# yijingru/KG_Instance_Segmentation

Hardware: AMD Instinct MI355X
Metric: imgs/s (train fwd+bwd) at 512x512 (higher is better)
Workload: dtype forward: f32-tolerance, hi + lo f16 planes (22 significant bits), 3 MFMA products / backward: f16 single planes, 1 MFMA product; f16 MFMA, fp32 accumulate; 1 GPU; KGnet train step fwd(dec+seg)+4xDetectionLossAll+SEG_loss+bwd+Adam, batch 8/GPU 3x512x512, 300 boxes/img, full HIP path; precision_policy=fp32, global_batch=8, parallelism=dp1, loss_readback=every step (train.py:156), grad_overflow=False

## Files before the change

include/kgnet_hip.h:

```cpp
#ifndef KGNET_HIP_H
#define KGNET_HIP_H
#ifdef __cplusplus
extern "C" {
#endif

typedef struct kg_planes {
    int a_planes, a_pstride;
    int b_planes, b_pstride;
    int c_planes, c_pstride;
    int y_planes, y_pstride;
    int w_planes;
    int reserved_;
    const float* scale;
    const float* oscale;
} kg_planes_t;

int kg_rows_format(void);

const char* kg_last_error(void);
const char* kg_last_kernel(void);
int kg_version(void);
int kg_device_arch(char* out, int cap);
int kg_tr_probe(void* out_u16x256, void* stream);
int kg_f64_probe(const double* a, const double* b, double* out5n, int n, void* stream);

int kg_conv2d_igemm(const void* x, const void* w, const float* bias, void* y, float* y_f32, const void* res,
                    const void* mask, const int* rowdesc, int M, int H, int W, int OH, int OW, int cin_pad, int ldx,
                    int Cout, int ldy, int ldres, int ldmask, int K, int KH, int KW, int stride, int pad, int dil,
                    int mode, int relu, int f32_C, int tile, const kg_planes_t* planes, void* stream);
int kg_conv2d_halo(const void* x, const void* w, const float* bias, void* y, float* y_f32, const void* res,
                   const void* mask, int N, int H, int W, int cin_pad, int ldx, int Cout, int ldy, int ldres, int ldmask,
                   int K, int KS, int flip, int relu, int f32_C, int wc, const int* tiletab, int ntiles, int total_rows,
                   const kg_planes_t* planes, void* stream);
int kg_conv2d_halo_heads2(const void* x, const void* w, const float* bias64, const int* vmap, float* kp, float* sh, float* md,
                          int N, int H, int W, int C, int ldx, int K, int kp_sigmoid, const kg_planes_t* planes, void* stream);
int kg_conv3x3_c64(const void* x, const void* w, const float* bias, void* y, const void* res, const void* mask, int N, int H, int W,
                   int ldx, int Cout, int ldy, int ldres, int ldmask, int K, int flip, int relu, const int* tiletab16, int ntiles,
                   void* stream);
int kg_conv7_narrow(const void* x, const void* w, void* y, const void* mask, int N, int H, int W, int ldx, int chan_lo, int chan_slot, int Cout, int ldy,
                    int ldmask, int K, int flip, void* stream);
int kg_conv3x3_ws(const void* x, const void* w, const float* bias, void* y, int N, int H, int W, int ldx, int ldy, int K, int relu,
                  const int* tiletab8, int ntiles, const kg_planes_t* planes, void* stream);
int kg_conv1x1(const void* x, const void* w, const float* bias, void* y, const void* res, const void* mask, long M, int K,
               int wK, int ldx, int Cout, int ldy, int ldres, int ldmask, int relu, void* stream);
int kg_pack_weight(const float* w, void* dst, int Cout, int Cin, int KH, int KW, int K, int cin_pad, int row0, int c0,
                   int transposed, int x_planes, int w_planes, void* stream);
int kg_pack_weight_rows(const float* w, void* dst, int Cout, int Cin, int KH, int KW, int K, int cin_pad, const int* rowmap,
                        int c0, int x_planes, int w_planes, int tap_stride, void* stream);
int kg_pack_weight_narrow(const float* w, void* dst, int Cout, int Cin, int KH, int KW, int K, int row0, int c0, int tap_stride, int tap_pitch,
                          void* stream);
int kg_pack_weight_batch(const void* jobs, int njobs, int total_blocks, void* stream);
int kg_im2col_small(const void* x, void* out, int N, int H, int W, int OH, int OW, int KH, int KW, int stride, int pad, int cin,
                    int ldx, int Kpad, void* stream);
int kg_conv2d_wgrad(const void* x, const void* dy, float* dwp, const int* rowdesc, int M, int H, int W, int OH, int OW,
                    int ldx, int lddy, int Cin, int Cout, int cin_lim, int cout_lim, int KH, int KW, int stride, int pad,
                    int dil, int mode, int nsplit, long split_stride, const kg_planes_t* planes, void* stream);
int kg_conv2d_wgrad_halo(const void* x, const void* dy, float* dwp, int N, int H, int W, int ldx, int lddy, int Cin, int Cout,
                         int cin_lim, int cout_lim, int KS, int nsplit, long split_stride, const int* tiletab16, int ntiles,
                         float* dbp, const kg_planes_t* planes, void* stream);
int kg_bias_grad_final(const float* part, float* db, int nsplit, int C, int accumulate, void* stream);
int kg_wgrad_reduce(const float* part, float* grad_oihw, int Cout, int Cin, int KH, int KW, int nsplit, long split_stride,
                    int accumulate, void* stream);
int kg_wgrad_reduce_multi(const float* part, float* const* grads_oihw, const int* counts, int ngrads, int Cin, int KH, int KW,
                          int nsplit, long split_stride, int accumulate, void* stream);
int kg_wgrad_reduce_bias(const float* part, float* const* grads_oihw, const int* counts, int ngrads, int Cin, int KH, int KW,
                         int nsplit, long split_stride, int accumulate, const float* bias_part, float* db, int bias_C, void* stream);
int kg_wgrad_reduce_defer(int on);
int kg_wgrad_reduce_pending(void);
int kg_wgrad_reduce_flush(void* stream);
int kg_bias_grad(const void* dy, float* db, float* scratch, int scratch_floats, int M, int C, int ld, int accumulate,
                 void* stream);
int kg_set_wgrad_tr(int use_transpose_read);

int kg_img_pack(const float* img_nchw, void* out_rows8, int ldout, int N, int C, int H, int W, const kg_planes_t* planes, void* stream);
int kg_bn_stats_train(const void* x, int ldx, int M, int C, const float* gamma, const float* beta, float* running_mean,
                      float* running_var, float momentum, float eps, float* mean_out, float* invstd_out, float* scale,
                      float* shift, float* scratch, int scratch_floats, const kg_planes_t* planes, void* stream);
int kg_conv_stats_begin(float* part, long cap_floats);
int kg_conv_stats_end(int* nb);
int kg_bn_finalize_train(const float* part, int nb, int M, int C, const float* gamma, const float* beta, float* running_mean,
                         float* running_var, float momentum, float eps, float* mean_out, float* invstd_out, float* scale,
                         float* shift, void* stream);
int kg_bn_scale_shift_eval(int C, const float* gamma, const float* beta, const float* running_mean,
                           const float* running_var, float eps, float* scale, float* shift, void* stream);
int kg_bn_apply(const void* x, int ldx, const float* scale, const float* shift, const void* res, int ldres, void* y,
                int ldy, int M, int C, int relu, const kg_planes_t* planes, void* stream);
int kg_bn_bwd(const void* x, int ldx, const void* dy, int lddy, const float* gamma, const float* mean,
              const float* invstd, float* dgamma, float* dbeta, int accumulate, void* dx, int lddx, int M, int C,
              float* scratch, int scratch_floats, const float* parts, int nb_parts, const float* parts_scale,
              const kg_planes_t* planes, void* stream);
int kg_bn_bwd_frozen(const void* x, int ldx, const void* dy, int lddy, const float* scale, const float* running_mean,
                     const float* running_var, float eps, float* dgamma, float* dbeta, int accumulate, void* dx, int lddx,
                     int M, int C, float* scratch, int scratch_floats, const kg_planes_t* planes, void* stream);
int kg_conv_bstats_begin(float* part, long cap_floats, const void* x, int ldx, int x_planes, int x_pstride, const float* mean,
                         const float* invstd);
int kg_maxpool3s2_fwd(const void* x, int ldx, void* y, int ldy, void* argmax_u8, int N, int H, int W, int C, const kg_planes_t* planes, void* stream);
int kg_maxpool3s2_bwd(const void* x, int ldx, const void* dy, int lddy, void* dx, int lddx, const void* argmax_u8, int N, int H, int W, int C,
                      const kg_planes_t* planes, void* stream);
int kg_bilinear_fwd(const void* x, int ldx, void* y, int ldy, int N, int IH, int IW, int OH, int OW, int C,
                    const int* boxdesc, const int* row2box, long total_out_rows, const kg_planes_t* planes, void* stream);
int kg_bilinear_bwd(const void* dy, int lddy, void* dx, int lddx, int N, int IH, int IW, int OH, int OW, int C,
                    const int* boxdesc, const int* row2box, long total_in_rows, const void* mask, int ldmask,
                    const kg_planes_t* planes, void* stream);
int kg_add_rows(const void* a, int lda, const void* b, int ldb, const void* mask, int ldm, void* y, int ldy, long M,
                int C, const float* scale, const float* scale2, const kg_planes_t* planes, void* stream);
int kg_sigmoid_inplace(float* x, long n, void* stream);
int kg_grad_pack(const float* g_nchw, const float* prob, void* out_rows, int N, int C, int H, int W, int ld, int cpad,
                 const kg_planes_t* planes, void* stream);
int kg_grad_pack3(const float* g0_nchw, const float* g1_nchw, const float* g2_nchw, const float* prob0, void* out_rows, int N, int C0, int C1, int C2,
                  int H, int W, int ld, int pad0, int pad1, int pad2, const kg_planes_t* planes, void* stream);

int kg_detection_loss_fwd(const float* kp, const float* sh, const float* md, const float* gt, int N, int H, int W,
                          float kp_radius, const float* den_override, float* scratch, int scratch_floats, float* out8,
                          void* stream);
int kg_detection_loss_bwd(const float* kp, const float* sh, const float* md, const float* gt, int N, int H, int W,
                          float kp_radius, const float* fin8, const float* grad_out, float* g_kp, float* g_sh,
                          float* g_md, void* stream);
int kg_seg_loss(const float* prob, const void* tgt_u8, const int* patches, const void* pairs, int npatches, float* part,
                float* out1, const float* grad_out, float* gprob, void* stream);

int kg_postproc_timing_begin(void);
int kg_postproc_timing_end(float* ms4);
long kg_postproc_workspace_bytes(int H, int W, int peak_cap, int skel_cap);
int kg_postproc_scale(const float* kp, const float* soff, const float* mid, int H, int W, double thresh, void* ws,
                      long ws_bytes, int peak_cap, int skel_cap, double* skel, int* nskel, double* heat_out,
                      double* blur_out, int* peaks_out, double* peak_conf_out, int* npeaks_out, void* stream);
int kg_skeleton_boxes(const double* skel, const int* nskel, int skel_cap, double scale, int do_refine, double* boxes,
                      int* nbox, int box_cap, void* stream);
int kg_nms(const double* boxes, const int* nbox, int box_cap, double thresh, void* ws, long ws_bytes, double* out,
           int* nkeep, void* stream);

long kg_postproc_batch_workspace_bytes(int N, int H, int W, int peak_cap, int skel_cap);
int kg_postproc_batch(const float* kp, const float* soff, const float* mid, int N, int H, int W, double thresh, void* ws,
                      long ws_bytes, int peak_cap, int skel_cap, double* skel, int* nskel, void* stream);
int kg_skeleton_boxes_batch(int N, int nscales, const double* const* skel, const int* const* nskel, const int* skel_cap,
                            const double* scale, int do_refine, double* boxes, int* nbox, int box_cap, void* stream);
long kg_nms_batch_workspace_bytes(int N, int box_cap);
int kg_nms_batch(int N, const double* boxes, const int* nbox, int box_cap, double thresh, void* ws, long ws_bytes, double* out,
                 int* nkeep, void* stream);

int kg_gt_maps(const float* kps, int n, int H, int W, float* out, void* stream);

int kg_sp_image(const void* imgs, int N, int H, int W, float* out, void* stream);
int kg_sp_warp_masks(const void* imgs, const int* inst_img, int ntot, int H, int W, void* out, int* box, void* stream);
int kg_sp_boxes(const void* imgs, int N, const int* box, int ntot, int kp_radius, int* counts, float* gtb, float* kp, int* keep,
                void* stream);

int kg_adam_step(const void* jobs, int njobs, int total_blocks, float beta1, float beta2, float eps, float step_size, float bc2_sqrt,
                 float weight_decay, void* stream);

int kg_host_crop_masks(const float* const* masks, const int* work, int nwork, int H, int W, unsigned char* out);
int kg_crop_masks(const void* masks, const int* work, int nwork, int H, int W, void* out, void* stream);
int kg_host_tile_table(const int* h, const int* w, const long* row0, int nb, int th, int tw, int* out, int cap);
int kg_host_bin_csr(const int* tab, int nb, int BS, int BY, int BX, int nbins, int* bin_start, int* bin_boxes, int cap);
int kg_host_match_boxes(const float* pb, int P, const float* gb, int G, int gstride, float thresh, int* pairs, int cap, int* count);

int kg_mask_areas(const void* masks, int n, long ld, int* area, void* stream);
int kg_mask_inter_pairs(const void* a, const void* b, const int* pairs, int npairs, long ld, int* inter, void* stream);

long kg_mask_bits_ld(int H, int W);
int kg_mask_pack_bits(const void* masks, int src_is_f32, int n, int H, int W, void* words, long ld_words, void* stream);
int kg_mask_unpack_bits(const void* words, long ld_words, int n, int H, int W, void* out, int out_is_u8, void* stream);
int kg_bitmask_areas(const void* words, int n, long ld_words, int* area, void* stream);
int kg_bitmask_inter_pairs(const void* a, int na, const void* b, int nb, const int* pairs, int npairs, long ld_words, int* inter,
                           void* stream);
int kg_instance_labels(const void* words, long ld_words, int n, const int* row_start, int nimg, int H, int W, const int* ids, int* labels,
                       long long* table, void* stream);
int kg_instance_overlay(const void* image, const void* words, long ld_words, int n, const int* row_start, int nimg, int H, int W,
                        const double* colors, double alpha, void* out, void* stream);

int kg_seg_build_rows(const int* boxtab8, int nb, int* rowdesc, int* row2box, int* srcrow, void* stream);
int kg_seg_build_rows_levels(int nlev, const int* const* boxtab8, const int* nb, int* const* rowdesc, int* const* row2box, int* const* srcrow,
                             void* stream);
int kg_rows_gather(const void* src, int ldsrc, const int* srcrow, void* dst, int lddst, long nrows, int C, void* stream);
int kg_rows_gather_planes(const void* src, int ldsrc, int src_pstride, const int* srcrow, void* dst, int lddst, int dst_pstride, long nrows, int C,
                          int P, void* stream);
int kg_seg_conv3_c1(const void* x, int ldx, int C, const float* w, const float* bias, const int* rowdesc, long M, float* y,
                    const kg_planes_t* planes, void* stream);
int kg_f32_to_bf16_rows(const float* acc, void* out, int C, long rows, int ldout, const void* addto, int ldadd,
                        void* stream);
int kg_rows_gather_f32(const float* src, int ldsrc, const int* srcrow, void* dst, int lddst, long nrows, int C,
                       const kg_planes_t* planes, void* stream);
int kg_planes_to_f32(const void* x, int ldx, float* out, int ldout, long rows, int C, const kg_planes_t* planes, void* stream);
int kg_f32_to_planes(const float* acc, int ldacc, void* out, int ldout, const void* addto, int ldadd, long rows, int C,
                     const kg_planes_t* planes, void* stream);
int kg_crop_grad_reduce(const void* ga, int lda, const void* gb, int ldb, long rows_a, const int* boxtab, const int* bin_start,
                        const int* bin_boxes, int bin_size, int N, int H, int W, int C, float* out, void* out_rows, int ldout,
                        const kg_planes_t* planes, void* stream);


int kg_mask_paste(const float* flat, const int* dets, int nd, int input_h, int input_w, int image_h, int image_w,
                  float seg_thresh, void* out, int out_is_u8, void* stream);
int kg_mask_paste_bits(const float* flat, const int* dets, int nd, int input_h, int input_w, int image_h, int image_w,
                       float seg_thresh, void* words, long ld_words, void* stream);

int kg_grad_scale(const void* const* ptrs, const void* const* probs, const long* counts, int n, int target_log2, void* scratch, float* out, void* stream);
int kg_scale_tensors(const void* jobs, int njobs, int total_blocks, int* nonfinite, void* stream);
int kg_rows_rescale(void* g, int ld, long M, int C, int target_log2, const float* cum_in, float* cum_out, float* r_out, void* scratch,
                    const kg_planes_t* planes, void* stream);
int kg_rows_scale(void* g, int ld, long M, int C, const float* r, const float* r2, const kg_planes_t* planes, void* stream);
int kg_rows_scale_multi(const long* desc, int n, const float* r, const float* r2, void* stream);

#ifdef __cplusplus
}
#endif
#endif
```

kg_instance_segmentation_amd/_lib.py:

```python
import ctypes
import os

_HERE = os.path.dirname(os.path.abspath(__file__))
LIB_PATH = os.environ.get("KG_LIB_PATH") or os.path.join(_HERE, "libkgnet_hip.so")
LIB_F16_PATH = os.environ.get("KG_LIB_F16_PATH") or os.path.join(os.path.dirname(LIB_PATH), "libkgnet_hip_f16.so")

c_int, c_long, c_float, c_double, c_void_p = ctypes.c_int, ctypes.c_long, ctypes.c_float, ctypes.c_double, ctypes.c_void_p
P = c_void_p

_SIGS = {
    "kg_version": [],
    "kg_rows_format": [],
    "kg_grad_scale": [P, P, P, c_int, c_int, P, P, P],
    "kg_scale_tensors": [P, c_int, c_int, P, P],
    "kg_rows_rescale": [P, c_int, c_long, c_int, c_int, P, P, P, P, P, P],
    "kg_rows_scale": [P, c_int, c_long, c_int, P, P, P, P],
    "kg_rows_scale_multi": [P, c_int, P, P, P],
    "kg_device_arch": [ctypes.c_char_p, c_int],
    "kg_tr_probe": [P, P],
    "kg_conv2d_igemm": [P, P, P, P, P, P, P, P] + [c_int] * 21 + [P, P],
    "kg_conv2d_halo": [P, P, P, P, P, P, P] + [c_int] * 15 + [P, c_int, c_int, P, P],
    "kg_conv1x1": [P, P, P, P, P, P, c_long] + [c_int] * 8 + [P],
    "kg_conv3x3_c64": [P, P, P, P, P, P] + [c_int] * 11 + [P, c_int, P],
    "kg_conv3x3_ws": [P, P, P, P] + [c_int] * 7 + [P, c_int, P, P],
    "kg_pack_weight": [P, P] + [c_int] * 11 + [P],
    "kg_pack_weight_rows": [P, P] + [c_int] * 6 + [P, c_int, c_int, c_int, c_int, P],
    "kg_pack_weight_batch": [P, c_int, c_int, P],
    "kg_pack_weight_narrow": [P, P] + [c_int] * 9 + [P],
    "kg_conv7_narrow": [P, P, P, P] + [c_int] * 11 + [P],
    "kg_im2col_small": [P, P] + [c_int] * 12 + [P],
    "kg_conv2d_halo_heads2": [P, P, P, P, P, P, P] + [c_int] * 7 + [P, P],
    "kg_set_wgrad_tr": [c_int],
    "kg_conv2d_wgrad": [P, P, P, P] + [c_int] * 18 + [c_long, P, P],
    "kg_conv2d_wgrad_halo": [P, P, P] + [c_int] * 11 + [c_long, P, c_int, P, P, P],
    "kg_bias_grad_final": [P, P, c_int, c_int, c_int, P],
    "kg_wgrad_reduce": [P, P, c_int, c_int, c_int, c_int, c_int, c_long, c_int, P],
    "kg_wgrad_reduce_multi": [P, P, P, c_int, c_int, c_int, c_int, c_int, c_long, c_int, P],
    "kg_wgrad_reduce_bias": [P, P, P, c_int, c_int, c_int, c_int, c_int, c_long, c_int, P, P, c_int, P],
    "kg_wgrad_reduce_defer": [c_int],
    "kg_wgrad_reduce_pending": [],
    "kg_wgrad_reduce_flush": [P],
    "kg_bias_grad": [P, P, P, c_int, c_int, c_int, c_int, c_int, P],
    "kg_img_pack": [P, P, c_int, c_int, c_int, c_int, c_int, P, P],
    "kg_bn_stats_train": [P, c_int, c_int, c_int, P, P, P, P, c_float, c_float, P, P, P, P, P, c_int, P, P],
    "kg_bn_scale_shift_eval": [c_int, P, P, P, P, c_float, P, P, P],
    "kg_conv_stats_begin": [P, c_long],
    "kg_conv_bstats_begin": [P, c_long, P, c_int, c_int, c_int, P, P],
    "kg_conv_stats_end": [P],
    "kg_bn_finalize_train": [P, c_int, c_int, c_int, P, P, P, P, c_float, c_float, P, P, P, P, P],
    "kg_bn_apply": [P, c_int, P, P, P, c_int, P, c_int, c_int, c_int, c_int, P, P],
    "kg_bn_bwd": [P, c_int, P, c_int, P, P, P, P, P, c_int, P, c_int, c_int, c_int, P, c_int, P, c_int, P, P, P],
    "kg_bn_bwd_frozen": [P, c_int, P, c_int, P, P, P, c_float, P, P, c_int, P, c_int, c_int, c_int, P, c_int, P, P],
    "kg_maxpool3s2_fwd": [P, c_int, P, c_int, P, c_int, c_int, c_int, c_int, P, P],
    "kg_maxpool3s2_bwd": [P, c_int, P, c_int, P, c_int, P, c_int, c_int, c_int, c_int, P, P],
    "kg_bilinear_fwd": [P, c_int, P, c_int, c_int, c_int, c_int, c_int, c_int, c_int, P, P, c_long, P, P],
    "kg_bilinear_bwd": [P, c_int, P, c_int, c_int, c_int, c_int, c_int, c_int, c_int, P, P, c_long, P, c_int, P, P],
    "kg_add_rows": [P, c_int, P, c_int, P, c_int, P, c_int, c_long, c_int, P, P, P, P],
    "kg_detection_loss_fwd": [P, P, P, P, c_int, c_int, c_int, c_float, P, P, c_int, P, P],
    "kg_detection_loss_bwd": [P, P, P, P, c_int, c_int, c_int, c_float, P, P, P, P, P, P],
    "kg_seg_loss": [P, P, P, P, c_int, P, P, P, P, P],
    "kg_sigmoid_inplace": [P, c_long, P],
    "kg_grad_pack": [P, P, P, c_int, c_int, c_int, c_int, c_int, c_int, P, P],
    "kg_grad_pack3": [P, P, P, P, P] + [c_int] * 10 + [P, P],
    "kg_postproc_workspace_bytes": [c_int, c_int, c_int, c_int],
    "kg_postproc_scale": [P, P, P, c_int, c_int, c_double, P, c_long, c_int, c_int, P, P, P, P, P, P, P, P],
    "kg_postproc_timing_begin": [],
    "kg_postproc_timing_end": [P],
    "kg_skeleton_boxes": [P, P, c_int, c_double, c_int, P, P, c_int, P],
    "kg_nms": [P, P, c_int, c_double, P, c_long, P, P, P],
    "kg_postproc_batch_workspace_bytes": [c_int, c_int, c_int, c_int, c_int],
    "kg_postproc_batch": [P, P, P, c_int, c_int, c_int, c_double, P, c_long, c_int, c_int, P, P, P],
    "kg_skeleton_boxes_batch": [c_int, c_int, P, P, P, P, c_int, P, P, c_int, P],
    "kg_nms_batch_workspace_bytes": [c_int, c_int],
    "kg_nms_batch": [c_int, P, P, c_int, c_double, P, c_long, P, P, P],
    "kg_gt_maps": [P, c_int, c_int, c_int, P, P],
    "kg_sp_image": [P, c_int, c_int, c_int, P, P],
    "kg_sp_warp_masks": [P, P, c_int, c_int, c_int, P, P, P],
    "kg_sp_boxes": [P, c_int, P, c_int, c_int, P, P, P, P, P],
    "kg_adam_step": [P, c_int, c_int, c_float, c_float, c_float, c_float, c_float, c_float, P],
    "kg_host_crop_masks": [P, P, c_int, c_int, c_int, P],
    "kg_crop_masks": [P, P, c_int, c_int, c_int, P, P],
    "kg_host_match_boxes": [P, c_int, P, c_int, c_int, c_float, P, c_int, P],
    "kg_host_tile_table": [P, P, P, c_int, c_int, c_int, P, c_int],
    "kg_host_bin_csr": [P, c_int, c_int, c_int, c_int, c_int, P, P, c_int],
    "kg_mask_areas": [P, c_int, c_long, P, P],
    "kg_mask_inter_pairs": [P, P, P, c_int, c_long, P, P],
    "kg_mask_bits_ld": [c_int, c_int],
    "kg_mask_pack_bits": [P, c_int, c_int, c_int, c_int, P, c_long, P],
    "kg_mask_unpack_bits": [P, c_long, c_int, c_int, c_int, P, c_int, P],
    "kg_bitmask_areas": [P, c_int, c_long, P, P],
    "kg_bitmask_inter_pairs": [P, c_int, P, c_int, P, c_int, c_long, P, P],
    "kg_instance_labels": [P, c_long, c_int, P, c_int, c_int, c_int, P, P, P, P],
    "kg_instance_overlay": [P, P, c_long, c_int, P, c_int, c_int, c_int, P, c_double, P, P],
    "kg_f64_probe": [P, P, P, c_int, P],
    "kg_seg_build_rows": [P, c_int, P, P, P, P],
    "kg_seg_build_rows_levels": [c_int, P, P, P, P, P, P],
    "kg_rows_gather": [P, c_int, P, P, c_int, c_long, c_int, P],
    "kg_rows_gather_planes": [P, c_int, c_int, P, P, c_int, c_int, c_long, c_int, c_int, P],
    "kg_seg_conv3_c1": [P, c_int, c_int, P, P, P, c_long, P, P, P],
    "kg_f32_to_bf16_rows": [P, P, c_int, c_long, c_int, P, c_int, P],
    "kg_rows_gather_f32": [P, c_int, P, P, c_int, c_long, c_int, P, P],
    "kg_planes_to_f32": [P, c_int, P, c_int, c_long, c_int, P, P],
    "kg_f32_to_planes": [P, c_int, P, c_int, P, c_int, c_long, c_int, P, P],
    "kg_mask_paste": [P, P, c_int, c_int, c_int, c_int, c_int, c_float, P, c_int, P],
    "kg_mask_paste_bits": [P, P, c_int, c_int, c_int, c_int, c_int, c_float, P, c_long, P],
    "kg_crop_grad_reduce": [P, c_int, P, c_int, c_long, P, P, P, c_int, c_int, c_int, c_int, c_int, P, P, c_int, P, P],
}
_RESTYPE = {"kg_postproc_workspace_bytes": c_long, "kg_postproc_batch_workspace_bytes": c_long, "kg_nms_batch_workspace_bytes": c_long,
            "kg_mask_bits_ld": c_long}
SYMBOLS = tuple(_SIGS) + ("kg_last_error", "kg_last_kernel")

_lib = None
_lib_f16 = None


class KGLibraryError(RuntimeError):
    pass


def _open(path, must_have_all):
    if not os.path.exists(path):
        raise KGLibraryError(
            f"{path} is missing: build it with `python -m kg_instance_segmentation_amd.build` "
            "(hipcc --offload-arch=gfx950).  There is no CPU fallback for the KGnet hot path.")
    lib = ctypes.CDLL(path)
    lib.kg_last_error.restype = ctypes.c_char_p
    lib.kg_last_error.argtypes = []
    lib.kg_last_kernel.restype = ctypes.c_char_p
    lib.kg_last_kernel.argtypes = []
    for name, args in _SIGS.items():
        if must_have_all:
            fn = getattr(lib, name)
        else:
            fn = getattr(lib, name, None)
            if fn is None:
                continue
        fn.argtypes = args
        fn.restype = _RESTYPE.get(name, c_int)
    return lib


def load(fmt=0):
    global _lib, _lib_f16
    if fmt:
        if _lib_f16 is None:
            lib = _open(LIB_F16_PATH, False)
            if lib.kg_rows_format() != 1:
                raise KGLibraryError(f"{LIB_F16_PATH} is not the half-precision build (kg_rows_format() != 1)")
            _lib_f16 = lib
        return _lib_f16
    if _lib is None:
        _lib = _open(LIB_PATH, True)
    return _lib


def call(name, *args, fmt=0):
    lib = load(fmt)
    rc = getattr(lib, name)(*args)
    if rc != 0:
        raise KGLibraryError(f"{name} failed ({rc}): {lib.kg_last_error().decode()}")


def last_kernel(fmt=0):
    return load(fmt).kg_last_kernel().decode()


_RAW_STREAM = None


def stream_ptr():
    global _RAW_STREAM
    import torch
    if _RAW_STREAM is None:
        _RAW_STREAM = getattr(torch._C, "_cuda_getCurrentRawStream", False)
    if _RAW_STREAM:
        return c_void_p(_RAW_STREAM(torch.cuda.current_device()))
    return c_void_p(torch.cuda.current_stream().cuda_stream)


def ptr(t):
    return None if t is None else c_void_p(t.data_ptr())
```

kg_instance_segmentation_amd/csrc/wgrad_halo.hip:

```cpp
#include "kg_common.h"
#include <stdlib.h>
#include <type_traits>
#include <utility>

struct WgHaloArgs {
    const bf16_t* x; const bf16_t* dy; float* dwp;
    const int4* tiletab;
    int ntiles;
    int N, H, W, tiles_x, tiles_y, ldx, lddy;
    int Cin, Cout, cin_lim, cout_lim, nsplit;
    long split_stride;
    float* dbp;
    WgPairs wp;
};

typedef __attribute__((address_space(3))) bf16x4 lds_bf16x4;
#ifndef KG_WG_LOOKAHEAD
#define KG_WG_LOOKAHEAD 2
#endif
__device__ __forceinline__ int dyf(int r) { return ((r >> 1) & 1) | (((r >> 4) & 1) << 1); }

template <int KS, int CIF>
struct WgGeom {
    static constexpr int PAD = KS / 2, HWD = 16 + KS - 1, T = KS * KS;
    static constexpr int XB = 32 * CIF;
    static constexpr int RAW = HWD * XB;
    static constexpr int PITCH = ((RAW - 128 + 255) / 256) * 256 + 128;
    static constexpr int DY_BYTES = 256 * 128, X_BYTES = HWD * PITCH, BUF = DY_BYTES + X_BYTES;
    static constexpr int UNITS = T * CIF, UPW = (UNITS + 7) / 8;
};

__device__ uint4 kg_wg_zero_line[8];

template <int OFF>
__device__ __forceinline__ void lds_rd_tr64(bf16x4& d, unsigned addr) {
    asm volatile("ds_read_b64_tr_b16 %0, %1 offset:%2" : "=v"(d) : "v"(addr), "n"(OFF));
}
template <int N>
__device__ __forceinline__ void lgkm_wait_n() { asm volatile("s_waitcnt lgkmcnt(%0)" ::"n"(N) : "memory"); }
__device__ __forceinline__ void tie(bf16x4& v) { asm volatile("" : "+v"(v)); }

template <int KS, int CIF, int NCF = 4, bool BIAS = false>
__global__ __launch_bounds__(512) void wgrad_halo_kernel(const WgHaloArgs a) {
    using GE = WgGeom<KS, CIF>;
    constexpr int PAD = GE::PAD, HWD = GE::HWD, T = GE::T, XB = GE::XB, PITCH = GE::PITCH;
    constexpr int DY_BYTES = GE::DY_BYTES, BUF = GE::BUF, UNITS = GE::UNITS, UPW = GE::UPW;
    constexpr int DQ = 256 * 8 / 512;
    constexpr int XROW = PITCH / 16, XREAL = HWD * 2 * CIF, XSL = HWD * XROW, XQ = (XSL + 511) / 512;
    static_assert(PITCH % 16 == 0 && BUF % 16 == 0 && DY_BYTES % 1024 == 0, "16-byte LDS-direct destinations");
    extern __shared__ __attribute__((aligned(16))) unsigned char smem[];

    const int tid = threadIdx.x, lane = tid & 63, wave = tid >> 6;
    const int wave_u = __builtin_amdgcn_readfirstlane(wave);
    const int n_ci_tiles = (a.cin_lim + 16 * CIF - 1) / (16 * CIF);
    int blk = blockIdx.x, split = blockIdx.y;
    if ((gridDim.y & 7) == 0) {
        const int L = blockIdx.y * gridDim.x + blockIdx.x;
        const int xcd = L & 7, slot = L >> 3;
        blk = slot % gridDim.x; split = (slot / gridDim.x) * 8 + xcd;
    } else if (((gridDim.x * gridDim.y) & 7) == 0 && gridDim.x >= 16) {
        const int L = blockIdx.y * gridDim.x + blockIdx.x;
        const int per = (gridDim.x * gridDim.y) >> 3;
        const int j = (L & 7) * per + (L >> 3);
        const int per_co = n_ci_tiles * gridDim.y;
        const int cob = j / per_co, rem = j - cob * per_co;
        split = rem / n_ci_tiles;
        blk = cob * n_ci_tiles + (rem - split * n_ci_tiles);
    }
    const int ci0 = (blk % n_ci_tiles) * 16 * CIF, co0 = (blk / n_ci_tiles) * 64;
    const int G = lane >> 4, i16 = lane & 15;

    f32x4 acc[UPW][NCF];
#pragma unroll
    for (int q = 0; q < UPW; ++q)
#pragma unroll
        for (int c = 0; c < NCF; ++c) acc[q][c] = f32x4{0.f, 0.f, 0.f, 0.f};
    constexpr int BW = UNITS % 8, BQ = UNITS / 8;
    static_assert(BQ < UPW, "no free unit slot for the bias-gradient unit");
    const bool do_bias = BIAS && ci0 == 0 && wave == BW;
    f32x4 accb[BIAS ? NCF : 1];
#pragma unroll
    for (int c = 0; c < (BIAS ? NCF : 1); ++c) accb[c] = f32x4{0.f, 0.f, 0.f, 0.f};
    bf16x8 ones;
#pragma unroll
    for (int e = 0; e < 8; ++e) ones[e] = (kg_h16)1.0f;

    const unsigned lds0 = lds_addr(smem);
    unsigned ay[NCF][2];
#pragma unroll
    for (int h = 0; h < 2; ++h) {
        const int r = (G & 1) * 16 + (G >> 1) * 8 + h * 4 + (i16 >> 2);
#pragma unroll
        for (int c = 0; c < NCF; ++c) ay[c][h] = lds0 + r * 128 + ((c ^ dyf(r)) * 32) + (i16 & 3) * 8;
    }
    unsigned bx[UPW][2];
#pragma unroll
    for (int q = 0; q < UPW; ++q) {
        int u = wave + 8 * q;
        if (u >= UNITS) u = UNITS - 1;
        const int tap = u / CIF, f = u - tap * CIF;
        const int ky = tap / KS, kx = tap - ky * KS;
#pragma unroll
        for (int h = 0; h < 2; ++h) {
            const int xh = (G >> 1) * 8 + h * 4 + (i16 >> 2) + kx;
            const int unit = CIF == 1 ? 0 : (f ^ (xh & (CIF - 1)));
            bx[q][h] = lds0 + DY_BYTES + ((G & 1) + ky) * PITCH + xh * XB + unit * 32 + (i16 & 3) * 8;
        }
    }

    const int tiles_plane = a.tiletab ? a.ntiles : a.N * a.tiles_x * a.tiles_y;
    const int tiles_total = a.wp.n * tiles_plane;

    int dy_p[DQ];
#pragma unroll
    for (int k = 0; k < DQ; ++k) {
        const int e = tid + k * 512, r = e >> 3, pc = e & 7;
        const int cp = (((pc >> 1) ^ dyf(r)) << 1) | (pc & 1);
        dy_p[k] = (r >> 4) | ((r & 15) << 8) | ((co0 + cp * 8 < a.cout_lim ? cp : 255) << 16);
    }
    int x_p[XQ];
#pragma unroll
    for (int k = 0; k < XQ; ++k) {
        const int e = tid + k * 512;
        const int hy = e / XROW, w = e - hy * XROW;
        const int hx = w / (2 * CIF), c = w - hx * (2 * CIF);
        const int unit = CIF == 1 ? 0 : ((c >> 1) ^ (hx & (CIF - 1)));
        const int sp = unit * 2 + (c & 1);
        const int fl = ((e < XSL && w < XREAL) ? 1 : 0) | ((ci0 + sp * 8 < a.cin_lim) ? 2 : 0);
        x_p[k] = ((hy - PAD + 8) & 255) | (((hx - PAD + 8) & 255) << 8) | (sp << 16) | (fl << 24);
    }
    const bf16_t* zline = reinterpret_cast<const bf16_t*>(kg_wg_zero_line);
    auto stage = [&](int vt, int buf) {
        const int pr = vt / tiles_plane, t = vt - pr * tiles_plane;
        int oy0, ox0, Hd, Wd; long rowbase;
        if (a.tiletab) {
            const int4 tt = a.tiletab[t];
            rowbase = tt.x; Hd = tt.y >> 16; Wd = tt.y & 0xffff; oy0 = tt.z >> 16; ox0 = tt.z & 0xffff;
        } else {
            int bt = t;
            const int tx = bt % a.tiles_x; bt /= a.tiles_x;
            const int ty = bt % a.tiles_y; const int n = bt / a.tiles_y;
            oy0 = ty * 16; ox0 = tx * 16; Hd = a.H; Wd = a.W; rowbase = (long)n * a.H * a.W;
        }
        const long base = rowbase + (long)oy0 * Wd + ox0;
        const bf16_t* dyb = a.dy + a.wp.doff[pr] + base * a.lddy;
        const bf16_t* xb = a.x + a.wp.xoff[pr] + base * a.ldx;
        const int hrem = Hd - oy0, wrem = Wd - ox0;
        unsigned char* sy = smem + buf * BUF;
        unsigned char* sx = sy + DY_BYTES;
        int lz = 0;
        asm volatile("" : "+v"(lz));
#pragma unroll
        for (int k = 0; k < DQ; ++k) {
            const int dp = dy_p[k] | lz;
            const int ry = dp & 255, rx = (dp >> 8) & 255, cp = dp >> 16;
            const bf16_t* src = zline;
            if (ry < hrem && rx < wrem && cp != 255) src = dyb + (long)(ry * Wd + rx) * a.lddy + co0 + cp * 8;
            __builtin_amdgcn_global_load_lds((const __attribute__((address_space(1))) void*)src,
                                             (__attribute__((address_space(3))) void*)(sy + (k * 512 + wave_u * 64) * 16), 16, 0, 0);
        }
#pragma unroll
        for (int k = 0; k < XQ; ++k) {
            if (x_p[k] & (1 << 24)) {
                const int xp = x_p[k] | lz;
                const int hy = (xp & 255) - 8, hx = ((xp >> 8) & 255) - 8, sp = (xp >> 16) & 255;
                const bf16_t* src = zline;
                if ((unsigned)(oy0 + hy) < (unsigned)Hd && (unsigned)(ox0 + hx) < (unsigned)Wd && (xp & (2 << 24)))
                    src = xb + (long)(hy * Wd + hx) * a.ldx + ci0 + sp * 8;
                __builtin_amdgcn_global_load_lds((const __attribute__((address_space(1))) void*)src,
                                                 (__attribute__((address_space(3))) void*)(sx + (k * 512 + wave_u * 64) * 16), 16, 0, 0);
            }
        }
    };

    auto rdA = [&](auto sc, bf16x4 (&f)[NCF][2]) {
        constexpr int S = decltype(sc)::value;
#pragma unroll
        for (int c = 0; c < NCF; ++c) { lds_rd_tr64<S * 32 * 128>(f[c][0], ay[c][0]); lds_rd_tr64<S * 32 * 128>(f[c][1], ay[c][1]); }
    };
    auto rdB = [&](auto sc, auto qc, bf16x4 (&f)[2]) {
        constexpr int S = decltype(sc)::value, Q = decltype(qc)::value;
        lds_rd_tr64<S * 2 * PITCH>(f[0], bx[Q][0]); lds_rd_tr64<S * 2 * PITCH>(f[1], bx[Q][1]);
    };
    auto cat = [](const bf16x4 (&f)[2]) { return __builtin_shufflevector(f[0], f[1], 0, 1, 2, 3, 4, 5, 6, 7); };

    int t = split;
    int cur = 0;
    if (t < tiles_total) stage(t, 0);
    for (; t < tiles_total; t += a.nsplit) {
        __syncthreads();
        const int tn = t + a.nsplit;
        if (tn < tiles_total && wave_u < 4) stage(tn, cur ^ 1);
        constexpr int LA = KG_WG_LOOKAHEAD;
        bf16x4 fa[2][NCF][2], fb[LA + 1][2];
        constexpr int NU = 8 * UPW;
        auto issue = [&](auto ic) {
            constexpr int I = decltype(ic)::value, S = I / UPW, Q = I % UPW;
            if constexpr (Q == 0) rdA(std::integral_constant<int, S>{}, fa[S & 1]);
            rdB(std::integral_constant<int, S>{}, std::integral_constant<int, Q>{}, fb[I % (LA + 1)]);
        };
        [&]<int... Ds>(std::integer_sequence<int, Ds...>) { (issue(std::integral_constant<int, Ds>{}), ...); }(std::make_integer_sequence<int, LA>{});
        auto step = [&](auto ic) {
            constexpr int I = decltype(ic)::value, S = I / UPW, Q = I % UPW;
            constexpr int ahead = []() { int n = 0; for (int d = 1; d <= LA; ++d) if (I + d < NU) n += 2 + ((I + d) % UPW == 0 ? 2 * NCF : 0); return n; }();
            if constexpr (I + LA < NU) issue(std::integral_constant<int, I + LA>{});
            lgkm_wait_n<ahead>();
            if constexpr (Q == 0) {
#pragma unroll
                for (int c = 0; c < NCF; ++c) { tie(fa[S & 1][c][0]); tie(fa[S & 1][c][1]); }
                if (BIAS && do_bias) {
#pragma unroll
                    for (int c = 0; c < (BIAS ? NCF : 1); ++c) accb[c] = KG_MFMA16(cat(fa[S & 1][c]), ones, accb[c]);
                }
            }
            tie(fb[I % (LA + 1)][0]); tie(fb[I % (LA + 1)][1]);
            if (Q < UNITS / 8 || wave + 8 * Q < UNITS) {
                const bf16x8 bfr = cat(fb[I % (LA + 1)]);
#pragma unroll
                for (int c = 0; c < NCF; ++c) acc[Q][c] = KG_MFMA16(cat(fa[S & 1][c]), bfr, acc[Q][c]);
            }
            __builtin_amdgcn_sched_barrier(0);
            if constexpr (I == 3 * UPW) {
                if (tn < tiles_total && wave_u >= 4) stage(tn, cur ^ 1);
                __builtin_amdgcn_sched_barrier(0);
            }
        };
        [&]<int... Is>(std::integer_sequence<int, Is...>) { (step(std::integral_constant<int, Is>{}), ...); }(std::make_integer_sequence<int, NU>{});
        {
            const int delta = cur ? -BUF : BUF;
#pragma unroll
            for (int c = 0; c < NCF; ++c) { ay[c][0] += delta; ay[c][1] += delta; }
#pragma unroll
            for (int q = 0; q < UPW; ++q) { bx[q][0] += delta; bx[q][1] += delta; }
            cur ^= 1;
        }
    }

    if (BIAS && do_bias && i16 == 0) {
#pragma unroll
        for (int c = 0; c < (BIAS ? NCF : 1); ++c)
#pragma unroll
            for (int r = 0; r < 4; ++r) {
                const int co = co0 + c * 16 + G * 4 + r;
                if (co < a.Cout) a.dbp[(long)split * a.Cout + co] = accb[c][r];
            }
    }
    float* out = a.dwp + (long)split * a.split_stride;
#pragma unroll
    for (int q = 0; q < UPW; ++q) {
        const int u = wave + 8 * q;
        if (u >= UNITS) continue;
        const int tap = u / CIF, f = u - tap * CIF;
        const int ci = ci0 + f * 16 + i16;
#pragma unroll
        for (int c = 0; c < NCF; ++c)
#pragma unroll
            for (int r = 0; r < 4; ++r) {
                const int co = co0 + c * 16 + G * 4 + r;
                if (co < a.Cout && ci < a.Cin) out[((long)co * T + tap) * a.Cin + ci] = acc[q][c][r];
            }
    }
}

template <int KS, int CIF, int NCF = 4, bool BIAS = false>
static int launch_wg(const WgHaloArgs& a, hipStream_t st) {
    constexpr int smem = 2 * WgGeom<KS, CIF>::BUF;
    static KgPerDevice attr_done;
    if (attr_done.first()) {
        KG_HIP(hipFuncSetAttribute((const void*)wgrad_halo_kernel<KS, CIF, NCF, BIAS>, hipFuncAttributeMaxDynamicSharedMemorySize, smem));
    }
    const int n_ci = (a.cin_lim + 16 * CIF - 1) / (16 * CIF), n_co = (a.cout_lim + 63) / 64;
    hipLaunchKernelGGL((wgrad_halo_kernel<KS, CIF, NCF, BIAS>), dim3(n_ci * n_co, a.nsplit), dim3(512), smem, st, a);
    KG_CHECK_LAUNCH("wgrad_halo");
    KG_KNAME(kname, "wgrad_halo_kernel<%d, %d, %d, %s>", KS, CIF, NCF, BIAS ? "true" : "false");
    kg_note_kernel(kname);
    return KG_OK;
}

extern "C" int kg_conv2d_wgrad_halo(const void* x, const void* dy, float* dwp, int N, int H, int W, int ldx, int lddy,
                                    int Cin, int Cout, int cin_lim, int cout_lim, int KS, int nsplit, long split_stride,
                                    const int* tiletab, int ntiles, float* dbp, const kg_planes_t* planes, void* stream) {
    WgHaloArgs a;
    memset(&a, 0, sizeof(a));
    const kg_planes_t pp = kg_planes_or_default(planes);
    KG_CHECK_ARG(kg_planes_ok(pp), "kg_conv2d_wgrad_halo: bad kg_planes_t");
    a.wp = kg_make_wgpairs(pp.a_planes, pp.a_pstride, pp.b_planes, pp.b_pstride);
    KG_CHECK_ARG(!dbp || a.wp.n == 1, "kg_conv2d_wgrad_halo: the fused bias gradient needs single-plane operands");
    KG_CHECK_ARG(x && dy && dwp, "kg_conv2d_wgrad_halo: null pointer");
    KG_CHECK_ARG(KS == 3 || KS == 7, "kg_conv2d_wgrad_halo: kernel size must be 3 or 7");
    KG_CHECK_ARG(ldx % 8 == 0 && lddy % 8 == 0 && cin_lim % 8 == 0 && cout_lim % 8 == 0, "kg_conv2d_wgrad_halo: ld/lim must be multiples of 8");
    KG_CHECK_ARG(nsplit >= 1 && ((tiletab && ntiles > 0) || (N > 0 && H > 0 && W > 0)), "kg_conv2d_wgrad_halo: bad sizes");
    a.x = (const bf16_t*)x; a.dy = (const bf16_t*)dy; a.dwp = dwp; a.N = N; a.H = H; a.W = W;
    a.tiles_x = kg_cdiv(W, 16); a.tiles_y = kg_cdiv(H, 16); a.ldx = ldx; a.lddy = lddy; a.Cin = Cin; a.Cout = Cout;
    a.cin_lim = cin_lim; a.cout_lim = cout_lim; a.nsplit = nsplit; a.split_stride = split_stride;
    a.tiletab = (const int4*)tiletab; a.ntiles = ntiles; a.dbp = dbp;
    hipStream_t st = (hipStream_t)stream;
    if (KS == 7) {
        if (dbp) {
            if (cout_lim <= 16 && cin_lim >= 32) return launch_wg<7, 2, 1, true>(a, st);
            if (cout_lim <= 16) return launch_wg<7, 1, 1, true>(a, st);
            if (cout_lim <= 48) return launch_wg<7, 1, 3, true>(a, st);
            return launch_wg<7, 1, 4, true>(a, st);
        }
        if (cout_lim <= 16) return launch_wg<7, 1, 1>(a, st);
        if (cout_lim <= 48) return launch_wg<7, 1, 3>(a, st);
        return launch_wg<7, 1>(a, st);
    }
    if (dbp) return cout_lim <= 16 ? launch_wg<3, 4, 1, true>(a, st) : launch_wg<3, 4, 4, true>(a, st);
    if (cout_lim <= 16) return launch_wg<3, 4, 1>(a, st);
    return launch_wg<3, 4>(a, st);
}
```

Before: 131.7 imgs/s.

## Add 4-wave 7x7 wgrad halo kernel with 96-wide Cout tiles and interleaved staging

Adds a new 256-thread weight-gradient kernel for dense 7x7 convolutions. Each block covers 96 output channels (six 16-wide fragments) and 13 taps per wave. Global-to-LDS staging of the next tile is interleaved between MFMA instructions under explicit scheduling barriers and LDS wait counts, and the grid is remapped across XCDs. The dispatcher picks this kernel automatically when Cout is at least 96, the map is large and the CU wave-count heuristic favours it, and KG_WGRAD7_W4=0 disables it. In exchange it uses many accumulator registers, tight hand scheduling and a larger LDS footprint per block.

```diff
diff --git a/include/kgnet_hip.h b/include/kgnet_hip.h
--- a/include/kgnet_hip.h
+++ b/include/kgnet_hip.h
@@ -58,6 +58,9 @@
 int kg_conv2d_wgrad_halo(const void* x, const void* dy, float* dwp, int N, int H, int W, int ldx, int lddy, int Cin, int Cout,
                          int cin_lim, int cout_lim, int KS, int nsplit, long split_stride, const int* tiletab16, int ntiles,
                          float* dbp, const kg_planes_t* planes, void* stream);
+int kg_conv2d_wgrad_halo7_w4(const void* x, const void* dy, float* dwp, int N, int H, int W, int ldx, int lddy, int Cin, int Cout,
+                             int cin_lim, int cout_lim, int KS, int nsplit, long split_stride, const int* tiletab16, int ntiles,
+                             float* dbp, const kg_planes_t* planes, void* stream);
 int kg_bias_grad_final(const float* part, float* db, int nsplit, int C, int accumulate, void* stream);
 int kg_wgrad_reduce(const float* part, float* grad_oihw, int Cout, int Cin, int KH, int KW, int nsplit, long split_stride,
                     int accumulate, void* stream);
diff --git a/kg_instance_segmentation_amd/_lib.py b/kg_instance_segmentation_amd/_lib.py
--- a/kg_instance_segmentation_amd/_lib.py
+++ b/kg_instance_segmentation_amd/_lib.py
@@ -33,6 +33,7 @@
     "kg_set_wgrad_tr": [c_int],
     "kg_conv2d_wgrad": [P, P, P, P] + [c_int] * 18 + [c_long, P, P],
     "kg_conv2d_wgrad_halo": [P, P, P] + [c_int] * 11 + [c_long, P, c_int, P, P, P],
+    "kg_conv2d_wgrad_halo7_w4": [P, P, P] + [c_int] * 11 + [c_long, P, c_int, P, P, P],
     "kg_bias_grad_final": [P, P, c_int, c_int, c_int, P],
     "kg_wgrad_reduce": [P, P, c_int, c_int, c_int, c_int, c_int, c_long, c_int, P],
     "kg_wgrad_reduce_multi": [P, P, P, c_int, c_int, c_int, c_int, c_int, c_long, c_int, P],
diff --git a/kg_instance_segmentation_amd/csrc/wgrad_halo.hip b/kg_instance_segmentation_amd/csrc/wgrad_halo.hip
--- a/kg_instance_segmentation_amd/csrc/wgrad_halo.hip
+++ b/kg_instance_segmentation_amd/csrc/wgrad_halo.hip
@@ -277,9 +277,284 @@
     return KG_OK;
 }
 
-extern "C" int kg_conv2d_wgrad_halo(const void* x, const void* dy, float* dwp, int N, int H, int W, int ldx, int lddy,
-                                    int Cin, int Cout, int cin_lim, int cout_lim, int KS, int nsplit, long split_stride,
-                                    const int* tiletab, int ntiles, float* dbp, const kg_planes_t* planes, void* stream) {
+struct Wg4Geom {
+    static constexpr int NCF = 6, UPW = 13, NU = 8 * UPW, LA = 2, QA0 = 4;
+    static constexpr int T = 49, HWD = WgGeom<7, 1>::HWD, PITCH = WgGeom<7, 1>::PITCH;
+    static constexpr int DYROW = NCF * 32, DY_BYTES = 256 * DYROW;
+    static constexpr int DQ = 256 * (DYROW / 16) / 256;
+    static constexpr int XROW = PITCH / 16, XSL = HWD * XROW, XQ = (XSL + 255) / 256, NP = DQ + XQ;
+    static constexpr int X_BYTES = XQ * 256 * 16, BUF = DY_BYTES + X_BYTES;
+    static constexpr int QV = 3;
+    static constexpr int STAGE_EVERY = 2;
+    static_assert(QA0 + NCF - 1 <= UPW - LA, "the dY^T fragments of k-step s+1 are issued before the X^T reads of its first unit");
+    static_assert((NP - 1) * STAGE_EVERY < NU, "all staging pieces fit into one tile");
+    static_assert(T <= 4 * UPW && T / 4 < UPW && 2 * BUF <= 160 * 1024 && BUF % 16 == 0 && DY_BYTES % 1024 == 0, "geometry");
+    static constexpr bool apart(int J) { return J / UPW + 1 < 8 && J % UPW >= QA0 && J % UPW < QA0 + NCF; }
+    static constexpr int issued_in(int J) { return (apart(J) ? 2 : 0) + (J + LA < NU ? 2 : 0); }
+    static constexpr int ahead(int I) {
+        int n = I < LA ? 2 * (LA - 1 - I) : 0;
+        for (int J = (I - LA + 1 > 0 ? I - LA + 1 : 0); J <= I; ++J) n += issued_in(J);
+        return n;
+    }
+};
+
+#ifdef KG_F16
+#define KG_MFMA16_ASM "v_mfma_f32_16x16x32_f16"
+#else
+#define KG_MFMA16_ASM "v_mfma_f32_16x16x32_bf16"
+#endif
+template <bool VG>
+__device__ __forceinline__ void wg4_mfma(f32x4& acc, const bf16x8& af, const bf16x8& bf) {
+    if constexpr (VG) asm(KG_MFMA16_ASM " %0, %1, %2, %0" : "+v"(acc) : "v"(af), "v"(bf));
+    else asm(KG_MFMA16_ASM " %0, %1, %2, %0" : "+a"(acc) : "v"(af), "v"(bf));
+}
+
+template <int NCF_, bool BIAS>
+__global__ __launch_bounds__(256) void wgrad_halo7_w4_kernel(const WgHaloArgs a) {
+    using GE = Wg4Geom;
+    static_assert(NCF_ == GE::NCF, "one geometry: 6 co-fragments");
+    constexpr int KS = 7, PAD = 3, T = GE::T, PITCH = GE::PITCH, NCF = GE::NCF, UPW = GE::UPW, NU = GE::NU, LA = GE::LA;
+    constexpr int DYROW = GE::DYROW, DY_BYTES = GE::DY_BYTES, BUF = GE::BUF, DQ = GE::DQ, XROW = GE::XROW, XSL = GE::XSL, XQ = GE::XQ;
+    extern __shared__ __attribute__((aligned(16))) unsigned char smem[];
+
+    const int tid = threadIdx.x, lane = tid & 63, wave = tid >> 6;
+    const int wave_u = __builtin_amdgcn_readfirstlane(wave);
+    const int n_ci_tiles = (a.cin_lim + 15) / 16;
+    int blk = blockIdx.x, split = blockIdx.y;
+    if ((gridDim.y & 7) == 0) {
+        const int L = blockIdx.y * gridDim.x + blockIdx.x;
+        const int xcd = L & 7, slot = L >> 3;
+        blk = slot % gridDim.x; split = (slot / gridDim.x) * 8 + xcd;
+    } else if (((gridDim.x * gridDim.y) & 7) == 0 && gridDim.x >= 16) {
+        const int L = blockIdx.y * gridDim.x + blockIdx.x;
+        const int per = (gridDim.x * gridDim.y) >> 3;
+        const int j = (L & 7) * per + (L >> 3);
+        const int per_co = n_ci_tiles * gridDim.y;
+        const int cob = j / per_co, rem = j - cob * per_co;
+        split = rem / n_ci_tiles;
+        blk = cob * n_ci_tiles + (rem - split * n_ci_tiles);
+    }
+    const int ci0 = (blk % n_ci_tiles) * 16, co0 = (blk / n_ci_tiles) * (16 * NCF);
+    const int G = lane >> 4, i16 = lane & 15;
+
+    f32x4 acc[UPW][NCF];
+#pragma unroll
+    for (int q = 0; q < UPW; ++q)
+#pragma unroll
+        for (int c = 0; c < NCF; ++c) acc[q][c] = f32x4{0.f, 0.f, 0.f, 0.f};
+    const bool do_bias = BIAS && ci0 == 0 && wave_u == 1;
+    bf16x8 alt;
+#pragma unroll
+    for (int e = 0; e < 8; ++e) alt[e] = (kg_h16)(do_bias ? 1.0f : 0.0f);
+
+    const unsigned lds0 = lds_addr(smem);
+    const int r0 = (G & 1) * 16 + (G >> 1) * 8 + (i16 >> 2);
+    unsigned aye = lds0 + r0 * DYROW + (G & 1) * 32 + (i16 & 3) * 8;
+    unsigned ayo = lds0 + r0 * DYROW + (1 - (G & 1)) * 32 + (i16 & 3) * 8;
+    unsigned bx[UPW];
+#pragma unroll
+    for (int q = 0; q < UPW; ++q) {
+        int u = wave + 4 * q;
+        if (u >= T) u = T - 1;
+        const int ky = u / KS, kx = u - ky * KS;
+        bx[q] = lds0 + DY_BYTES + ((G & 1) + ky) * PITCH + ((G >> 1) * 8 + (i16 >> 2) + kx) * 32 + (i16 & 3) * 8;
+    }
+
+    const int tiles_total = a.N * a.tiles_x * a.tiles_y;
+
+    int dy_p[3];
+#pragma unroll
+    for (int m = 0; m < 3; ++m) {
+        const int i = m * 64 + lane, rx = i / (DYROW / 16), pc = i - rx * (DYROW / 16);
+        dy_p[m] = rx | (pc << 8);
+    }
+    int x_p[XQ];
+#pragma unroll
+    for (int k = 0; k < XQ; ++k) {
+        const int e = tid + k * 256;
+        const int hy = e / XROW, w = e - hy * XROW;
+        const int hx = w >> 1, sp = w & 1;
+        const int fl = (e < XSL ? 1 : 0) | ((ci0 + sp * 8 < a.cin_lim) ? 2 : 0);
+        x_p[k] = ((hy - PAD + 8) & 255) | (((hx - PAD + 8) & 255) << 8) | (sp << 16) | (fl << 24);
+    }
+    const bf16_t* zline = reinterpret_cast<const bf16_t*>(kg_wg_zero_line);
+    struct TileG { const bf16_t* dyb; const bf16_t* xb; int oy0, ox0, hrem, wrem; };
+    auto tile_geom = [&](int t) {
+        const int tx = t % a.tiles_x; t /= a.tiles_x;
+        const int ty = t % a.tiles_y; const int n = t / a.tiles_y;
+        TileG g;
+        g.oy0 = ty * 16; g.ox0 = tx * 16; g.hrem = a.H - g.oy0; g.wrem = a.W - g.ox0;
+        const long base = (long)n * a.H * a.W + (long)g.oy0 * a.W + g.ox0;
+        g.dyb = a.dy + a.wp.doff[0] + base * a.lddy;
+        g.xb = a.x + a.wp.xoff[0] + base * a.ldx;
+        return g;
+    };
+    struct StageSt { const bf16_t* src; int c0, c1; bool ok; };
+    auto stage_phase = [&](auto jc, auto pc, StageSt& st, const TileG& g, int buf) {
+        constexpr int J = decltype(jc)::value, PH = decltype(pc)::value;
+        if constexpr (J < DQ) {
+            const int ry = wave_u * 4 + J / 3;
+            if constexpr (PH == 0) {
+                int lz = 0;
+                asm volatile("" : "+v"(lz));
+                const int dp = dy_p[J % 3] | lz;
+                st.c0 = dp & 255; st.c1 = (dp >> 8) ^ (((J / 3) & 1) << 1);
+            } else if constexpr (PH == 1) {
+                st.ok = ry < g.hrem && st.c0 < g.wrem && co0 + st.c1 * 8 < a.cout_lim;
+                st.c0 += ry * a.W;
+            } else if constexpr (PH == 2) {
+                st.src = g.dyb + (long)st.c0 * a.lddy + co0 + st.c1 * 8;
+                asm volatile("" : "+v"(st.src));
+            } else if constexpr (PH == 3) {
+                st.src = st.ok ? st.src : zline;
+            } else if constexpr (PH == 4) {
+                __builtin_amdgcn_global_load_lds((const __attribute__((address_space(1))) void*)st.src,
+                                                 (__attribute__((address_space(3))) void*)(smem + buf * BUF + (wave_u * DQ + J) * 1024), 16, 0, 0);
+            }
+        } else {
+            constexpr int K = J - DQ;
+            if constexpr (PH == 0) {
+                int lz = 0;
+                asm volatile("" : "+v"(lz));
+                const int xp = x_p[K] | lz;
+                st.c0 = (xp & 255) - 8; st.c1 = ((xp >> 8) & 255) - 8;
+                st.ok = (xp >> 24) == 3;
+                st.src = g.xb + ci0 + ((xp >> 16) & 255) * 8;
+            } else if constexpr (PH == 1) {
+                st.ok = st.ok && (unsigned)(g.oy0 + st.c0) < (unsigned)a.H && (unsigned)(g.ox0 + st.c1) < (unsigned)a.W;
+                st.c0 = st.c0 * a.W + st.c1;
+            } else if constexpr (PH == 2) {
+                st.src += (long)st.c0 * a.ldx;
+                asm volatile("" : "+v"(st.src));
+            } else if constexpr (PH == 3) {
+                st.src = st.ok ? st.src : zline;
+            } else if constexpr (PH == 4) {
+                __builtin_amdgcn_global_load_lds((const __attribute__((address_space(1))) void*)st.src,
+                                                 (__attribute__((address_space(3))) void*)(smem + buf * BUF + DY_BYTES + (K * 256 + wave_u * 64) * 16), 16, 0, 0);
+            }
+        }
+    };
+    auto stage_piece = [&](auto jc, const TileG& g, int buf) {
+        StageSt st;
+        [&]<int... Ps>(std::integer_sequence<int, Ps...>) { (stage_phase(jc, std::integral_constant<int, Ps>{}, st, g, buf), ...); }(std::make_integer_sequence<int, 5>{});
+    };
+
+    auto rdA = [&](auto sc, auto cc, bf16x4 (&f)[NCF][2]) {
+        constexpr int S = decltype(sc)::value, C = decltype(cc)::value, OFF = S * 32 * DYROW + (C >> 1) * 64;
+        lds_rd_tr64<OFF>(f[C][0], (C & 1) ? ayo : aye); lds_rd_tr64<OFF + 4 * DYROW>(f[C][1], (C & 1) ? ayo : aye);
+    };
+    auto rdB = [&](auto ic, bf16x4 (&f)[2]) {
+        constexpr int I = decltype(ic)::value, S = I / UPW, Q = I % UPW;
+        lds_rd_tr64<S * 2 * PITCH>(f[0], bx[Q]); lds_rd_tr64<S * 2 * PITCH + 128>(f[1], bx[Q]);
+    };
+    auto cat = [](const bf16x4 (&f)[2]) { return __builtin_shufflevector(f[0], f[1], 0, 1, 2, 3, 4, 5, 6, 7); };
+
+    int t = split;
+    int cur = 0;
+    if (t < tiles_total) {
+        const TileG g = tile_geom(t);
+        [&]<int... Js>(std::integer_sequence<int, Js...>) { (stage_piece(std::integral_constant<int, Js>{}, g, 0), ...); }(std::make_integer_sequence<int, GE::NP>{});
+    }
+    for (; t < tiles_total; t += a.nsplit) {
+        __syncthreads();
+        const int tn = t + a.nsplit;
+        const bool nxt = tn < tiles_total;
+        const TileG gn = tile_geom(nxt ? tn : t);
+        __builtin_amdgcn_sched_barrier(0);
+        bf16x4 fa[2][NCF][2], fb[LA + 1][2];
+        [&]<int... Cs>(std::integer_sequence<int, Cs...>) { (rdA(std::integral_constant<int, 0>{}, std::integral_constant<int, Cs>{}, fa[0]), ...); }(std::make_integer_sequence<int, NCF>{});
+        [&]<int... Ds>(std::integer_sequence<int, Ds...>) { (rdB(std::integral_constant<int, Ds>{}, fb[Ds % (LA + 1)]), ...); }(std::make_integer_sequence<int, LA>{});
+        auto step = [&](auto ic) {
+            constexpr int I = decltype(ic)::value, S = I / UPW, Q = I % UPW;
+            if constexpr (GE::apart(I)) rdA(std::integral_constant<int, S + 1>{}, std::integral_constant<int, Q - GE::QA0>{}, fa[(S + 1) & 1]);
+            if constexpr (I + LA < NU) rdB(std::integral_constant<int, I + LA>{}, fb[(I + LA) % (LA + 1)]);
+            lgkm_wait_n<GE::ahead(I)>();
+            if constexpr (Q == 0) {
+#pragma unroll
+                for (int c = 0; c < NCF; ++c) { tie(fa[S & 1][c][0]); tie(fa[S & 1][c][1]); }
+            }
+            tie(fb[I % (LA + 1)][0]); tie(fb[I % (LA + 1)][1]);
+            bf16x8 bfr = cat(fb[I % (LA + 1)]);
+            if constexpr (Q == UPW - 1) {
+                bfr = wave_u == 0 ? bfr : alt;
+                asm volatile("s_nop 1" : "+v"(bfr));
+            }
+            constexpr bool STG = I % GE::STAGE_EVERY == 0 && I / GE::STAGE_EVERY < GE::NP;
+            StageSt st;
+            [&]<int... Cs>(std::integer_sequence<int, Cs...>) {
+                ([&] {
+                    wg4_mfma<(Q >= UPW - GE::QV)>(acc[Q][Cs], cat(fa[S & 1][Cs]), bfr);
+                    if constexpr (STG && Cs < 5) {
+                        __builtin_amdgcn_sched_barrier(0);
+                        stage_phase(std::integral_constant<int, I / GE::STAGE_EVERY>{}, std::integral_constant<int, Cs>{}, st, gn, cur ^ 1);
+                        __builtin_amdgcn_sched_barrier(0);
+                    }
+                }(), ...);
+            }(std::make_integer_sequence<int, NCF>{});
+            __builtin_amdgcn_sched_barrier(0);
+        };
+        [&]<int... Is>(std::integer_sequence<int, Is...>) { (step(std::integral_constant<int, Is>{}), ...); }(std::make_integer_sequence<int, NU>{});
+        {
+            const int delta = cur ? -BUF : BUF;
+            aye += delta; ayo += delta;
+#pragma unroll
+            for (int q = 0; q < UPW; ++q) bx[q] += delta;
+            cur ^= 1;
+        }
+    }
+    asm volatile("s_waitcnt vmcnt(0)\n\ts_nop 15\n\ts_nop 15" ::: "memory");
+
+    if (BIAS && do_bias && i16 == 0) {
+#pragma unroll
+        for (int c = 0; c < NCF; ++c)
+#pragma unroll
+            for (int r = 0; r < 4; ++r) {
+                const int co = co0 + c * 16 + G * 4 + r;
+                if (co < a.Cout) a.dbp[(long)split * a.Cout + co] = acc[UPW - 1][c][r];
+            }
+    }
+    float* out = a.dwp + (long)split * a.split_stride;
+#pragma unroll
+    for (int q = 0; q < UPW; ++q) {
+        const int tap = wave + 4 * q;
+        if (tap >= T) continue;
+        const int ci = ci0 + i16;
+#pragma unroll
+        for (int c = 0; c < NCF; ++c)
+#pragma unroll
+            for (int r = 0; r < 4; ++r) {
+                const int co = co0 + c * 16 + G * 4 + r;
+                if (co < a.Cout && ci < a.Cin) out[((long)co * T + tap) * a.Cin + ci] = acc[q][c][r];
+            }
+    }
+}
+
+template <bool BIAS>
+static int launch_wg7_w4(const WgHaloArgs& a, hipStream_t st) {
+    constexpr int smem = 2 * Wg4Geom::BUF;
+    static KgPerDevice attr_done;
+    if (attr_done.first()) {
+        KG_HIP(hipFuncSetAttribute((const void*)wgrad_halo7_w4_kernel<Wg4Geom::NCF, BIAS>, hipFuncAttributeMaxDynamicSharedMemorySize, smem));
+    }
+    const int n_ci = (a.cin_lim + 15) / 16, n_co = kg_cdiv(a.cout_lim, 16 * Wg4Geom::NCF);
+    hipLaunchKernelGGL((wgrad_halo7_w4_kernel<Wg4Geom::NCF, BIAS>), dim3(n_ci * n_co, a.nsplit), dim3(256), smem, st, a);
+    KG_CHECK_LAUNCH("wgrad_halo7_w4");
+    KG_KNAME(kname, "wgrad_halo7_w4_kernel<%d, %s>", Wg4Geom::NCF, BIAS ? "true" : "false");
+    kg_note_kernel(kname);
+    return KG_OK;
+}
+
+static bool wg7_w4_pays(const WgHaloArgs& a) {
+    static const int on = getenv("KG_WGRAD7_W4") ? atoi(getenv("KG_WGRAD7_W4")) : 1;
+    if (!on || a.tiletab || a.wp.n != 1 || a.cout_lim < 96 || (long)a.N * a.H * a.W < 16384) return false;
+    const long n_ci = (a.cin_lim + 15) / 16, cus = 256;
+    const long r8 = kg_cdiv(n_ci * kg_cdiv(a.cout_lim, 64) * a.nsplit, cus), r4 = kg_cdiv(n_ci * kg_cdiv(a.cout_lim, 96) * a.nsplit, cus);
+    return r4 * 96 <= r8 * 64;
+}
+
+static int wg_halo_dispatch(int w4, const void* x, const void* dy, float* dwp, int N, int H, int W, int ldx, int lddy,
+                            int Cin, int Cout, int cin_lim, int cout_lim, int KS, int nsplit, long split_stride,
+                            const int* tiletab, int ntiles, float* dbp, const kg_planes_t* planes, void* stream) {
     WgHaloArgs a;
     memset(&a, 0, sizeof(a));
     const kg_planes_t pp = kg_planes_or_default(planes);
@@ -295,7 +570,12 @@
     a.cin_lim = cin_lim; a.cout_lim = cout_lim; a.nsplit = nsplit; a.split_stride = split_stride;
     a.tiletab = (const int4*)tiletab; a.ntiles = ntiles; a.dbp = dbp;
     hipStream_t st = (hipStream_t)stream;
+    if (w4) {
+        KG_CHECK_ARG(KS == 7 && !tiletab && a.wp.n == 1, "kg_conv2d_wgrad_halo7_w4: dense 7x7 maps with single-plane operands only");
+        return dbp ? launch_wg7_w4<true>(a, st) : launch_wg7_w4<false>(a, st);
+    }
     if (KS == 7) {
+        if (wg7_w4_pays(a)) return dbp ? launch_wg7_w4<true>(a, st) : launch_wg7_w4<false>(a, st);
         if (dbp) {
             if (cout_lim <= 16 && cin_lim >= 32) return launch_wg<7, 2, 1, true>(a, st);
             if (cout_lim <= 16) return launch_wg<7, 1, 1, true>(a, st);
@@ -310,3 +590,15 @@
     if (cout_lim <= 16) return launch_wg<3, 4, 1>(a, st);
     return launch_wg<3, 4>(a, st);
 }
+
+extern "C" int kg_conv2d_wgrad_halo(const void* x, const void* dy, float* dwp, int N, int H, int W, int ldx, int lddy,
+                                    int Cin, int Cout, int cin_lim, int cout_lim, int KS, int nsplit, long split_stride,
+                                    const int* tiletab, int ntiles, float* dbp, const kg_planes_t* planes, void* stream) {
+    return wg_halo_dispatch(0, x, dy, dwp, N, H, W, ldx, lddy, Cin, Cout, cin_lim, cout_lim, KS, nsplit, split_stride, tiletab, ntiles, dbp, planes, stream);
+}
+
+extern "C" int kg_conv2d_wgrad_halo7_w4(const void* x, const void* dy, float* dwp, int N, int H, int W, int ldx, int lddy,
+                                        int Cin, int Cout, int cin_lim, int cout_lim, int KS, int nsplit, long split_stride,
+                                        const int* tiletab, int ntiles, float* dbp, const kg_planes_t* planes, void* stream) {
+    return wg_halo_dispatch(1, x, dy, dwp, N, H, W, ldx, lddy, Cin, Cout, cin_lim, cout_lim, KS, nsplit, split_stride, tiletab, ntiles, dbp, planes, stream);
+}
```

Measured after the change: 128.6 imgs/s. -2.3%, worse.
